# fnordware/j2k

Hardware: AMD Instinct MI355X
Metric: Mpixels/s encode, 8Kx8K 16-bit RGB, 5 DWT levels; DWT HBM GB/s vs roofline (higher is better)
Workload: dtype f32

## Files before the change

### j2k_amd/csrc/encoder.cpp

```cpp
#include <hip/hip_runtime.h>

#include <dlfcn.h>

#include <algorithm>
#include <atomic>
#include <chrono>
#include <condition_variable>
#include <functional>
#include <future>
#include <limits>
#include <cstdio>
#include <cstdlib>
#include <cstring>
#include <memory>
#include <mutex>
#include <thread>
#include <string>
#include <vector>

#include "common.h"
#include "geometry.h"
#include "kernels.h"
#include "tier2.h"
#include "jp2.h"
// ... 625 lines not shown
                hipStream_t side = coder_stream(e, 0);
                HIP_CHECK(hipEventRecord(e->rc_fixed, s));
                HIP_CHECK(hipStreamWaitEvent(side, e->rc_fixed, 0));
                HIP_CHECK(hipMemcpyAsync(e->h_passes.p, ta.pass_nmsedec, tt.h_passes_bytes(), hipMemcpyDeviceToHost, side));
                HIP_CHECK(hipEventRecord(e->rc_tables, side));
                pd.rc_tables_pending = true;
            }
            HIP_CHECK(hipMemcpyAsync(e->h_rc_bounds.p, ra.bounds, 3 * nb * sizeof(double), hipMemcpyDeviceToHost, s));
        }
    } else {
        pd.rc_device = false;
        if (cod.cblk_style && nb) {
            T1Args tf = ta;
            tf.first = 0; tf.nblks = (int)nb;
            launch_t1_rate_fixup(tf, s);
            e->h_passes.ensure(tt.h_rates_bytes());
            HIP_CHECK(hipMemcpyAsync(e->h_passes.p, ta.pass_rate, tt.h_rates_bytes(), hipMemcpyDeviceToHost, s));
        }
    }
    if (overlap_mq) dev.last_dense_done = e->k1_done;
    else HIP_CHECK(hipStreamSynchronize(s));
    dense.unlock();

    pd.active = true;
    pd.F = F; pd.nb1 = nb1; pd.framed = framed; pd.rate_control = rate_control; pd.dwt_bytes = dwt_bytes;
    pd.meta = meta; pd.dblk = dblk; pd.nl = NL;
}

std::vector<EncodeOut> encode_end(j2k_hip_encoder *e)
{
    Pending &pd = e->pend;
    if (!pd.active) throw Error(J2K_HIP_ERR_PARAM, "no encode in progress on this handle");
    if (pd.banded) throw Error(J2K_HIP_ERR_PARAM, "internal: a band-pipelined encode ends in encode_end_banded");
    pd.active = false;
    struct Leave {
        j2k_hip_encoder *e;
        ~Leave() { if (e->counted_inflight) { g_dev[e->device].inflight.fetch_sub(1); e->counted_inflight = false; } }
    } leave{e};
    HIP_CHECK(hipSetDevice(e->device));
    hipStream_t s = e->stream;
    const Geometry &g = e->geo;
    const Coding &cod = g.cod;
    const size_t F = pd.F, nb1 = pd.nb1, nb = nb1 * F;
    const bool framed = pd.framed, rate_control = pd.rate_control;
    const int NL = pd.nl;
    uint32_t *meta = pd.meta;
    const CblkDev *dblk = pd.dblk;
    const std::vector<CblkDev> &hblk = F > 1 ? e->h_blks_seq : e->h_blks;
    {
        Range r("j2k_hip wait t1");
        HIP_CHECK(hipStreamSynchronize(s));
    }
    const double t_t2 = now_ms();
    const T1Tables tt(nb);
    const uint32_t *hm = e->h_meta.as<uint32_t>();
    if (*tt.err(hm) != 0)
        throw Error(J2K_HIP_ERR_OVERFLOW, "Tier-1 kernel reported error " + std::to_string(*tt.err(hm)) +
                                              " (1: too many bit-planes, 2: decision buffer, 3: codeword buffer)");
    uint64_t nsym_total = 0;
    for (size_t i = 0; i < nb; ++i) nsym_total += tt.nsym(hm)[i];
    const size_t lead = main_header(cod).size() + jp2_file_header(cod, 0).size();
    std::vector<Tier2Plan> plans(F);
    std::vector<GatherPlan> lays(F);
    std::vector<size_t> plan_off(F), cs_off(F);
    size_t plan_total = 0, cs_total = 0;
    const size_t nbd = rate_control ? 0 : nb1;
    uint32_t guard = cod.guard;
    {
        Range r("j2k_hip tier2 host");
        for (size_t f = 0; f < F; ++f) {
            std::vector<CblkResult> res(nb1);
            const size_t b0 = f * nb1;
            for (size_t i = 0; i < nb1; ++i) res[i] = CblkResult{tt.numbps(hm)[b0 + i], tt.npasses(hm)[b0 + i], tt.len(hm)[b0 + i]};
            if (cod.cblk_style)
                for (size_t i = 0; i < nb1; ++i) res[i].rates = e->h_passes.as<uint32_t>() + tt.row(b0 + i);
            auto plan_frame = [&](const Geometry &gg) -> Tier2Plan {
                LayerAlloc alloc;
                if (rate_control) {
                    const uint32_t *hp = e->h_passes.as<uint32_t>();
                    const uint32_t *h_rate = tt.h_rate(hp) + tt.row(b0), *h_nmsedec = hp + tt.row(b0);
#ifdef J2K_ALLOC_DUMP
                    if (pd.rc_tables_pending) { HIP_CHECK(hipEventSynchronize(e->rc_tables)); pd.rc_tables_pending = false; }
                    if (const char *path = std::getenv("J2K_ALLOC_DUMP")) {
                        static bool dumped = false;
                        if (!dumped && f == 0) {
                            dumped = true;
                            if (FILE *fp = std::fopen(path, "wb")) {
                                const uint32_t head[10] = {(uint32_t)nb1, (uint32_t)kDevMaxPasses, cod.width, cod.height, cod.ncomp, cod.prec,
                                                           cod.reversible ? 1u : 0u, cod.numres, 1u << cod.cbw, 1u << cod.cbh};
                                std::fwrite(head, 4, 10, fp);
                                for (size_t i = 0; i < nb1; ++i) {
                                    const uint32_t r3[3] = {res[i].numbps, res[i].npasses, res[i].len};
                                    std::fwrite(r3, 4, 3, fp);
                                    std::fwrite(h_rate + tt.row(i), 4, res[i].npasses, fp);
                                    std::fwrite(h_nmsedec + tt.row(i), 4, res[i].npasses, fp);
                                }
                                std::fclose(fp);
                            }
                        }
                    }
#endif
                    std::unique_ptr<HipRateDevice> rdev;
                    if (pd.rc_device) rdev.reset(new HipRateDevice(e, tt));
                    const unsigned at = std::max(1u, std::min((unsigned)std::max(1, tuning().alloc_threads), std::thread::hardware_concurrency()));
                    if (nb1 >= 4096 && !(e->alloc_workers && e->alloc_workers->size() == at)) e->alloc_workers.reset(new Workers(at));
                    alloc = allocate_layers(gg, res, h_rate, reinterpret_cast<const int32_t *>(h_nmsedec), lead, at, rdev.get(), e->alloc_workers.get());
                }
                if (pd.rc_tables_pending) { HIP_CHECK(hipEventSynchronize(e->rc_tables)); pd.rc_tables_pending = false; }
                if (nb1 >= 4096 && !e->t2_workers) e->t2_workers.reset(new Workers(plan_threads()));
                return plan_codestream(gg, res, framed, framed, rate_control ? &alloc : nullptr, e->t2_workers.get());
            };
            guard = cod.guard;
            try { plans[f] = plan_frame(g); }
            catch (const GuardExcess &) {
                if (!cod.guard_auto) throw;
                guard = guard_bits_needed(g, res);
                plans[f] = plan_frame(with_guard_bits(g, guard));
            }
            lays[f] = GatherPlan(plans[f].blob.size(), plans[f].hdr_segs.size(), nbd, plans[f].body_segs.size());
            plan_off[f] = plan_total;
            plan_total += lays[f].total;
            cs_off[f] = cs_total;
            cs_total += round_up(plans[f].total_len + 64, 256);
        }
    }
    const double t_t2_end = now_ms();

    Range r_asm("j2k_hip assemble");
    e->h_plan.ensure(plan_total);
    e->plan.ensure(plan_total);
    e->cs.ensure(cs_total);
    std::vector<GatherArgs> gas(F);
    for (size_t f = 0; f < F; ++f) {
        const Tier2Plan &plan = plans[f];
        const size_t nh = plan.hdr_segs.size(), nseg = plan.body_segs.size();
        uint8_t *hp = e->h_plan.as<uint8_t>() + plan_off[f];
        std::memcpy(hp, plan.blob.data(), plan.blob.size());
        const GatherTables h = lays[f].tables(hp);
        for (size_t i = 0; i < nh; ++i) { h.hdr_dst[i] = plan.hdr_segs[i].dst; h.hdr_src[i] = plan.hdr_segs[i].src; h.hdr_len[i] = plan.hdr_segs[i].len; }
        if (nbd) std::memcpy(h.cblk_dst, plan.cblk_dst.data(), nbd * 8);
        for (size_t i = 0; i < nseg; ++i) {
            const BodySeg &b = plan.body_segs[i];
            h.seg_dst[i] = b.dst; h.seg_src[i] = hblk[f * nb1 + b.cblk].out_off + b.off; h.seg_len[i] = b.len;
        }
        GatherArgs &ga = gas[f];
        lays[f].fill(ga, e->plan.as<uint8_t>() + plan_off[f]);
        ga.dst = e->cs.as<uint8_t>() + cs_off[f];
        ga.out = e->out.as<uint8_t>(); ga.blks = dblk + f * nb1; ga.len = tt.len(meta) + f * nb1; ga.nblks = (int)nbd;
    }
    HIP_CHECK(hipMemcpyAsync(e->plan.p, e->h_plan.p, plan_total, hipMemcpyHostToDevice, s));
    for (size_t f = 0; f < F; ++f) launch_gather(gas[f], s);
    HIP_CHECK(hipEventRecord(e->ev[EV_GATHER], s));
    HIP_CHECK(hipStreamSynchronize(s));

    j2k_hip_stats &st = e->stats;
    st = j2k_hip_stats{};
    float ms = 0;
    HIP_CHECK(hipEventElapsedTime(&ms, e->ev[EV_START], e->ev[EV_UPLOAD])); st.ms_upload = ms;
    HIP_CHECK(hipEventElapsedTime(&ms, e->ev[EV_UPLOAD], e->ev[EV_FRONT])); st.ms_frontend = ms;
    HIP_CHECK(hipEventElapsedTime(&ms, e->ev[EV_FRONT], e->ev[EV_DWT])); st.ms_dwt = ms;
    HIP_CHECK(hipEventElapsedTime(&ms, e->ev[EV_DWT], e->ev[EV_T1])); st.ms_t1 = ms;
    if (tuning().level_events && F == 1) {
        for (int l = 0; l < NL; ++l) { HIP_CHECK(hipEventElapsedTime(&ms, e->lev[l], e->lev[l + 1])); e->level_ms[l] = ms; }
    } else if (NL > 0 && F == 1) {
        HIP_CHECK(hipEventElapsedTime(&ms, e->lev[0], e->lev[1])); e->level_ms[0] = ms;
        if (NL > 1) {
            HIP_CHECK(hipEventElapsedTime(&ms, e->lev[1], e->lev[NL]));
            for (int l = 1; l < NL; ++l) e->level_ms[l] = ms / (NL - 1);
        }
    } else if (NL > 0) {
        HIP_CHECK(hipEventElapsedTime(&ms, e->lev[0], e->lev[NL]));
        for (int l = 0; l < NL; ++l) e->level_ms[l] = ms / NL;
    }
    st.ms_t2_host = t_t2_end - t_t2;
    st.ms_assemble = now_ms() - t_t2_end;
    st.codestream_bytes = 0;
    for (const Tier2Plan &pl : plans) st.codestream_bytes += pl.total_len;
    st.num_codeblocks = nb;
    st.num_symbols = nsym_total;
    st.dwt_bytes = pd.dwt_bytes;
    st.ms_total = now_ms() - pd.t_begin;
    st.ms_after_upload = st.ms_total - st.ms_upload;
    std::vector<EncodeOut> outs(F);
    for (size_t f = 0; f < F; ++f) { outs[f].d_cs = e->cs.as<uint8_t>() + cs_off[f]; outs[f].len = (size_t)plans[f].total_len; }
    if (framed) e->last_guard = guard;
    return outs;
}



void frame_span(const Coding &cod, const j2k_hip_plane *planes, int y0, int y1, const uint8_t *&lo, const uint8_t *&hi)
{
    lo = hi = nullptr;
    for (uint32_t c = 0; c < cod.ncomp; ++c) {
        const j2k_hip_plane &p = planes[c];
        if (!p.base) throw Error(J2K_HIP_ERR_PARAM, "channel buffer is NULL");
        check_plane(cod, p);
        const uint8_t *b = static_cast<const uint8_t *>(p.base);
        const uint8_t *corners[4] = {b + (ptrdiff_t)y0 * p.rowbytes, b + (ptrdiff_t)(y1 - 1) * p.rowbytes,
                                     b + (ptrdiff_t)y0 * p.rowbytes + (ptrdiff_t)(cod.width - 1) * p.colbytes,
                                     b + (ptrdiff_t)(y1 - 1) * p.rowbytes + (ptrdiff_t)(cod.width - 1) * p.colbytes};
        for (const uint8_t *q : corners) {
            if (!lo || q < lo) lo = q;
            if (!hi || q + p.sample_bits / 8 > hi) hi = q + p.sample_bits / 8;
        }
    }
// ... 190 lines not shown
    HIP_CHECK(hipEventRecord(e->ev[EV_T1], s));

    pd.active = true;
    pd.F = 1; pd.nb1 = nb; pd.framed = true; pd.rate_control = false; pd.dwt_bytes = dwt_bytes;
    pd.meta = meta; pd.dblk = ta.blks; pd.nl = NL;
    pd.banded = true; pd.stages = NS; pd.bands = B; pd.ms_upload_host = up_ms;
    return true;
}

struct PieceWriter {
    j2k_hip_write_fn write; void *user; std::vector<uint8_t> &bounce; size_t fill = 0;
    static constexpr size_t kSmall = 256u << 10, kBounce = 4u << 20;
    void out(const uint8_t *p, size_t n) { if (n && write(user, p, n) != n) throw Error(J2K_HIP_ERR_SINK, "Error writing file"); }
    void flush() { if (fill) { out(bounce.data(), fill); fill = 0; } }
    void put(const uint8_t *p, size_t n)
    {
        if (n >= kSmall) { flush(); out(p, n); return; }
        if (bounce.size() < kBounce) bounce.resize(kBounce);
        if (fill + n > kBounce) flush();
        std::memcpy(bounce.data() + fill, p, n);
        fill += n;
    }
};

void encode_end_banded(j2k_hip_encoder *e, j2k_hip_write_fn write, void *user)
{
    Pending &pd = e->pend;
    if (!pd.active || !pd.banded) throw Error(J2K_HIP_ERR_PARAM, "no band-pipelined encode in progress on this handle");
    pd.active = false; pd.banded = false;
    struct Leave {
        j2k_hip_encoder *e;
        ~Leave() { if (e->counted_inflight) { g_dev[e->device].inflight.fetch_sub(1); e->counted_inflight = false; } }
    } leave{e};
    HIP_CHECK(hipSetDevice(e->device));
    const Geometry &g = e->geo;
    const BandSchedule &S = e->band;
    const size_t nb = pd.nb1;
    const int NS = pd.stages, B = pd.bands;
    const T1Tables tt(nb);
    const uint32_t *hm = e->h_meta.as<uint32_t>();
    std::vector<uint64_t> pack_off(nb);
    std::vector<CblkResult> res(nb);
    uint64_t early = 0, nsym_total = 0;
    std::mutex mu;
    std::condition_variable cv;
    uint32_t done_mask = 0;
    bool failed = false;
    const std::function<void(uint32_t)> before_res = [&](uint32_t r) {
        std::unique_lock<std::mutex> lk(mu);
        const uint32_t need = r < S.res_stages.size() ? S.res_stages[r] : 0u;
        cv.wait(lk, [&] { return failed || (done_mask & need) == need; });
        if (failed) throw Error(J2K_HIP_ERR_DEVICE, "the frame's stages did not complete");
    };
    if (nb >= 4096 && !e->t2_workers) e->t2_workers.reset(new Workers(plan_threads()));
    double t_t2 = 0, t_t2_end = 0;
    std::future<Tier2Plan> planner = std::async(std::launch::async, [&] {
        Range r("j2k_hip tier2 host");
        Tier2Plan pl = plan_codestream(g, res, true, true, nullptr, e->t2_workers.get(), &before_res);
        t_t2_end = now_ms();
        return pl;
    });
    auto abandon = [&] {
        { std::lock_guard<std::mutex> lk(mu); failed = true; }
        cv.notify_all();
        try { (void)planner.get(); } catch (...) {}
    };
    try {
        Range r("j2k_hip stages down");
        bool pending[j2k_hip_encoder::kMaxStages] = {};
        int remaining = NS;
        for (int k = 0; k < NS; ++k) pending[k] = true;
        while (remaining) {
            bool progress = false;
            for (int k = 0; k < NS; ++k) {
                if (!pending[k]) continue;
                const hipError_t q = hipEventQuery(e->stage_done[k]);
                if (q == hipErrorNotReady) continue;
                HIP_CHECK(q);
                const BandStage &st = S.stages[(size_t)k];
                uint64_t tot = 0;
                for (size_t n = st.blk_first; n < (size_t)st.blk_first + st.blk_count; ++n) {
                    pack_off[n] = tot; tot += tt.len(hm)[n]; nsym_total += tt.nsym(hm)[n];
                    res[S.perm[n]] = CblkResult{tt.numbps(hm)[n], tt.npasses(hm)[n], tt.len(hm)[n]};
                }
                if (tot) {
                    if (tot > e->out_bytes) throw Error(J2K_HIP_ERR_OVERFLOW, "internal: a stage's codewords exceed the arena");
                    e->h_stage_cs[k].ensure((size_t)tot);
                    HIP_CHECK(hipMemcpyAsync(e->h_stage_cs[k].p, e->cs.as<uint8_t>() + e->h_blks_band[st.blk_first].out_off, (size_t)tot, hipMemcpyDeviceToHost, coder_stream(e, 1)));
                }
                HIP_CHECK(hipEventRecord(e->stage_dl[k], coder_stream(e, 1)));
                if (st.band < B - 1) early += tot;
                { std::lock_guard<std::mutex> lk(mu); done_mask |= 1u << k; }
                cv.notify_all();
                pending[k] = false; --remaining; progress = true;
                if (remaining == 0) t_t2 = now_ms();
            }
            if (!progress) std::this_thread::sleep_for(std::chrono::microseconds(20));
        }
        HIP_CHECK(hipStreamSynchronize(e->stream));
    } catch (...) {
        abandon();
        throw;
    }
    if (*tt.err(hm) != 0) {
        abandon();
        throw Error(J2K_HIP_ERR_OVERFLOW, "Tier-1 kernel reported error " + std::to_string(*tt.err(hm)) +
                                              " (1: too many bit-planes, 2: decision buffer, 3: codeword buffer)");
    }
    Tier2Plan plan;
    uint32_t guard = g.cod.guard;
    try { plan = planner.get(); }
    catch (const GuardExcess &) {
        if (!g.cod.guard_auto) throw;
        Range r("j2k_hip tier2 host, guard bits");
        guard = guard_bits_needed(g, res);
        plan = plan_codestream(with_guard_bits(g, guard), res, true, true, nullptr, e->t2_workers.get());
        t_t2_end = now_ms();
    }
    struct Piece { uint64_t dst; const uint8_t *src; uint64_t len; int stage; };
    std::vector<Piece> hp, bp, all;
    hp.reserve(plan.hdr_segs.size()); bp.reserve(nb);
    for (const HeaderSeg &h : plan.hdr_segs) if (h.len) hp.push_back({h.dst, plan.blob.data() + h.src, h.len, -1});
    for (size_t i = 0; i < nb; ++i) {
        if (!res[i].len) continue;
        const size_t n = S.inv[i];
        const int k = (int)S.stage_of[n];
        const uint8_t *src = e->h_stage_cs[k].as<uint8_t>() + pack_off[n];
        if (!bp.empty() && bp.back().stage == k && bp.back().dst + bp.back().len == plan.cblk_dst[i] && bp.back().src + bp.back().len == src)
            bp.back().len += res[i].len;
        else bp.push_back({plan.cblk_dst[i], src, res[i].len, k});
    }
    auto by_dst = [](const Piece &a, const Piece &b) { return a.dst < b.dst; };
    if (!std::is_sorted(hp.begin(), hp.end(), by_dst)) std::sort(hp.begin(), hp.end(), by_dst);
    if (!std::is_sorted(bp.begin(), bp.end(), by_dst)) std::sort(bp.begin(), bp.end(), by_dst);
    all.resize(hp.size() + bp.size());
    std::merge(hp.begin(), hp.end(), bp.begin(), bp.end(), all.begin(), by_dst);
    {
        Range r("j2k_hip sink");
        PieceWriter w{write, user, e->bounce};
        bool arrived[j2k_hip_encoder::kMaxStages] = {};
        uint64_t pos = 0;
        double waited = 0;
        for (const Piece &pc : all) {
            if (pc.dst != pos) throw Error(J2K_HIP_ERR_PARAM, "internal: the file's pieces do not join up");
            if (pc.stage >= 0 && !arrived[pc.stage]) {
                const double tw = now_ms();
                HIP_CHECK(hipEventSynchronize(e->stage_dl[pc.stage]));
                waited += now_ms() - tw;
                arrived[pc.stage] = true;
            }
            w.put(pc.src, (size_t)pc.len);
            pos += pc.len;
        }
        w.flush();
        if (pos != plan.total_len) throw Error(J2K_HIP_ERR_PARAM, "internal: the file's pieces do not add up to its length");
        e->stats.ms_download = waited;
    }
    HIP_CHECK(hipStreamSynchronize(coder_stream(e, 1)));

    j2k_hip_stats &st = e->stats;
    const double waited = st.ms_download;
    st = j2k_hip_stats{};
    float ms = 0;
    HIP_CHECK(hipEventElapsedTime(&ms, e->ev[EV_START], e->ev[EV_T1]));
    st.ms_t1 = ms;
    st.ms_upload = pd.ms_upload_host;
    st.ms_t2_host = t_t2_end - t_t2;
    st.ms_download = waited;
    st.codestream_bytes = plan.total_len;
// ... 521 lines not shown
```

### j2k_amd/csrc/handle.h

```cpp
#pragma once

#include <hip/hip_runtime.h>

#include <atomic>
#include <chrono>
#include <cstdlib>
#include <future>
#include <memory>
#include <string>
#include <thread>
#include <vector>

#include "bands.h"
#include "common.h"
#include "geometry.h"
#include "kernels.h"
#include "table_layout.h"

namespace j2k_hip {

#define HIP_CHECK(expr)                                                                             \
    do {                                                                                            \
        hipError_t e_ = (expr);                                                                     \
        if (e_ != hipSuccess)                                                                       \
            throw Error(J2K_HIP_ERR_DEVICE, std::string(#expr) + ": " + hipGetErrorString(e_));     \
    } while (0)

struct DevBuf {
    void *p = nullptr;
    size_t cap = 0;
    DevBuf() = default;
    DevBuf(const DevBuf &) = delete;
    DevBuf &operator=(const DevBuf &) = delete;
    ~DevBuf() { release(); }
    void ensure(size_t n)
    {
        if (n <= cap) return;
        if (p) { (void)hipFree(p); p = nullptr; cap = 0; }
        const size_t want = n + n / 8 + 4096;
        if (hipMalloc(&p, want) != hipSuccess) {
            p = nullptr;
            throw Error(J2K_HIP_ERR_MEMORY, "hipMalloc of " + std::to_string(want) + " bytes failed");
        }
        cap = want;
    }
    void release() { if (p) (void)hipFree(p); p = nullptr; cap = 0; }
    template <typename T> T *as() const { return reinterpret_cast<T *>(p); }
};

struct PinnedBuf {
    void *p = nullptr;
    size_t cap = 0;
    PinnedBuf() = default;
    PinnedBuf(const PinnedBuf &) = delete;
    PinnedBuf &operator=(const PinnedBuf &) = delete;
    ~PinnedBuf() { release(); }
    void ensure(size_t n)
    {
        if (n <= cap) return;
        if (p) { (void)hipHostFree(p); p = nullptr; cap = 0; }
        const size_t want = n + n / 8 + 4096;
        if (hipHostMalloc(&p, want, hipHostMallocDefault) != hipSuccess) {
            p = nullptr;
            throw Error(J2K_HIP_ERR_MEMORY, "hipHostMalloc of " + std::to_string(want) + " bytes failed");
        }
        cap = want;
    }
    void release() { if (p) (void)hipHostFree(p); p = nullptr; cap = 0; }
    template <typename T> T *as() const { return reinterpret_cast<T *>(p); }
};

static_assert(kMaxPasses == kDevMaxPasses, "table_layout.h and the Tier-1 kernels agree on the passes per block");

inline unsigned plan_threads() { return std::max(1u, std::min(4u, std::thread::hardware_concurrency())); }

inline int hw_queues()
{
    static const int q = [] {
        const char *v = std::getenv("GPU_MAX_HW_QUEUES");
        const int n = v ? std::atoi(v) : 0;
        return n > 0 ? n : 4;
    }();
    return q;
}

inline double now_ms()
{
    using namespace std::chrono;
    return duration<double, std::milli>(steady_clock::now().time_since_epoch()).count();
}

enum { EV_START, EV_UPLOAD, EV_FRONT, EV_DWT, EV_T1, EV_GATHER, EV_DONE, EV_COUNT };

constexpr int kMaxLevels = 33;


}

struct Pending {
    bool active = false;
    double t_begin = 0;
    size_t F = 1, nb1 = 0;
    bool framed = true, rate_control = false;
    bool rc_device = false;
    bool rc_tables_pending = false;
    double dwt_bytes = 0;
    uint32_t *meta = nullptr;
    const j2k_hip::CblkDev *dblk = nullptr;
    int nl = 0;
    bool banded = false;
    int stages = 0, bands = 0;
    double ms_upload_host = 0, t_uploaded = 0;
};

struct j2k_hip_encoder {
    int device = 0;
    Pending pend;
    std::future<int> begin_job;
    std::atomic<bool> begin_async{false};
    j2k_hip_params begin_params = {};
    j2k_hip_plane begin_planes[4] = {};
    bool last_fused = false;
    j2k_hip::FrontendArgs last_fa = {};
    hipStream_t stream = nullptr;
    hipStream_t mqs[12] = {};
    hipEvent_t gev[12] = {};
    hipEvent_t mq_done[12] = {};
// ... 132 lines not shown
```

### j2k_amd/csrc/kernels.h

```cpp
#pragma once

#include <hip/hip_runtime.h>

#include <cstdint>

#include "rgba_plan.h"

namespace j2k_hip {

struct Tuning {
    int overlap = 1;
    int no_fuse = 0;
    int level_events = 0;
    int level1_dispatch_events = 1;
    int mq_prio = 1;
    int mq_yield = 2;
    int groups = 2;
    int alloc_threads = 8;
    int rate_dev = 0;
    int rate_dev_scan = 0;
    int mq_wait_us = 1500;
    int dwt_pairs = 2;
    int dwt_ppc = 0;
    int dwt_min_waves = 2048;
    int fused_wpb = 0;
    int fused_ppc = 0;
    int fused_generic = 0;
    int dwt_xcd = 1;
    int t1dec_tail = 1;
    int t1dec_lanes = 1;
    int decseq_group = 0;
    int bands = 0;
    int t1_sparse = 0;
};
Tuning &tuning();
int tune(const char *key, int value);
int get_tune(const char *key, int *value);

struct FrontendArgs {
    const uint8_t *src[4];
    long long colbytes[4], rowbytes[4];
    int sample_bytes[4];
    int src_depth[4];
    int ncomp;
    int width;
    int x0;
    int y0, y1;
    int dst_x0, dst_y0;
    int prec;
    int reversible, mct, promote;
    int interleaved;
    const uint8_t *pixel_base;
    int pixel_bytes;
    int chan_off[4];
    void *dst[4];
    long long dst_stride;
    const float *xyz_lin[3];
    const float *xyz_thr;
    float xyz_m[9];
};
void launch_frontend(const FrontendArgs &a, hipStream_t s);
void launch_frontend_sycc(const FrontendArgs &a, int sub_x, int sub_y, hipStream_t s);
void launch_frontend_xyz(const FrontendArgs &a, hipStream_t s);

constexpr int kCompareWords = 8;
constexpr int kCompareSets = 16;
struct CompareArgs {
    FrontendArgs src;
    int wide;
    const int *planes[4]; long long plane_stride; int plane_dc;
    const uint16_t *dec[4]; long long dec_stride[4]; int dec_sx[4], dec_sy[4];
    int ncomp, width, height;
    int slot[4];
    unsigned long long *acc;
};
void launch_compare(const CompareArgs &a, hipStream_t s);

struct DwtJob {
    long long src_off;
    long long ll_off;
    long long z_off;
    int rw, rh;
    int casx, casy;
    int px0, py0;
};
struct DwtLevelArgs {
// ... 202 lines not shown
```

### j2k_amd/csrc/tier2.cpp

```cpp
#include "tier2.h"
#include "cblk_style.h"
#include "jp2.h"

#include <algorithm>
#include <cstring>

namespace j2k_hip {
namespace {

struct ByteVec {
    std::vector<uint8_t> &v;
    void u8(unsigned x) { v.push_back((uint8_t)x); }
    void u16(unsigned x) { u8(x >> 8); u8(x & 0xff); }
    void u32(uint32_t x) { u16(x >> 16); u16(x & 0xffff); }
};

struct BitWriter {
    std::vector<uint8_t> &out;
    uint32_t buf = 0;
    int ct = 8;
    explicit BitWriter(std::vector<uint8_t> &o) : out(o) {}
    void byteout()
    {
        buf = (buf << 8) & 0xffff;
        ct = buf == 0xff00 ? 7 : 8;
        out.push_back((uint8_t)(buf >> 8));
    }
    void bit(unsigned b)
    {
        if (ct == 0) byteout();
        --ct;
        buf |= b << ct;
    }
    void bits(uint32_t v, int n) { for (int i = n - 1; i >= 0; --i) bit((v >> i) & 1); }
    void flush() { byteout(); if (ct == 7) byteout(); }
};

class TagTree {
    struct Node { int parent; int value, low; bool known; };
    std::vector<Node> n_;
  public:
    TagTree(uint32_t w, uint32_t h)
    {
        std::vector<std::pair<uint32_t, uint32_t>> dims;
        uint32_t cw = w, ch = h;
        size_t total = 0;
        while (true) {
            dims.push_back({cw, ch});
            total += (size_t)cw * ch;
            if ((size_t)cw * ch <= 1) break;
            cw = (cw + 1) / 2; ch = (ch + 1) / 2;
        }
        n_.assign(total, Node{-1, 999, 0, false});
        size_t base = 0;
        for (size_t l = 0; l + 1 < dims.size(); ++l) {
            const size_t next = base + (size_t)dims[l].first * dims[l].second;
            for (uint32_t y = 0; y < dims[l].second; ++y)
                for (uint32_t x = 0; x < dims[l].first; ++x)
// ... 707 lines not shown
        }
    };
    if (nt <= 1) packets_of(0); else workers->run(std::min(nt, std::max(1u, npackets)), packets_of);
    uint64_t total = m.committed_bytes;
    if (per_comp) for (uint32_t c = 0; c < m.ncomp; ++c) per_comp[c] = 0;
    for (uint32_t pr = 0; pr < m.pairs.size(); ++pr)
        for (uint32_t pi = m.pairs[pr].packet0; pi < m.pairs[pr].packet0 + m.pairs[pr].npackets; ++pi) {
            total += m.packet_total[pi];
            if (per_comp) per_comp[pr % m.ncomp] += m.packet_total[pi];
        }
    return total;
}

uint64_t TilePricer::committed() const { return p_->committed_bytes; }

uint32_t packet_block_bits(uint32_t np, uint32_t len)
{
    if (!np) return 0;
    BitRecorder r;
    count_numpasses(r, np);
    const int lnp = floorlog2(np);
    const int inc = std::max(0, floorlog2(len) + 1 - (3 + lnp));
    uint32_t bits = (uint32_t)r.n + (uint32_t)inc + 1u;
    return bits + (uint32_t)(3 + inc + lnp);
}

uint64_t TilePricer::tree_bits_bound(uint32_t comp) const
{
    const Impl &m = *p_;
    uint64_t bits = 0;
    for (uint32_t pr = comp; pr < m.pairs.size(); pr += m.ncomp)
        for (uint32_t pi = m.pairs[pr].packet0; pi < m.pairs[pr].packet0 + m.pairs[pr].npackets; ++pi) {
            ++bits;
            for (uint32_t ui = m.packets[pi].unit0; ui < m.packets[pi].unit0 + m.packets[pi].nunits; ++ui) {
            const Impl::Unit &u = m.units[ui];
        for (uint32_t i = u.node0; i < u.node1; ++i) {
            bits += 2;
            const int32_t par = m.parent[i];
            const int v = m.imsb[i].value, pv = par >= 0 ? m.imsb[(size_t)par].value : 0;
            if (v < 999) bits += (uint64_t)(v - pv) + 1u;
        }
            }
        }
    return bits;
}

void TilePricer::commit(const LayerAlloc &alloc, uint32_t layno)
{
    Impl &m = *p_;
    for (const Impl::Pair &pr : m.pairs) m.committed_bytes += m.walk_pair(pr, alloc, layno, m.incl.data(), m.imsb.data(), true);
    m.forget_candidate();
}

Tier2Plan plan_codestream(const Geometry &geo, const std::vector<CblkResult> &res, bool with_main_header,
                          bool with_eoc, const LayerAlloc *alloc, Workers *workers, const std::function<void(uint32_t)> *before_res)
{
    const Coding &cod = geo.cod;
    Tier2Plan plan;
    if (!alloc) plan.cblk_dst.assign(geo.cblks.size(), 0);
    std::vector<uint8_t> &blob = plan.blob;
    blob.reserve(geo.cblks.size() * 4 + 4096);
    uint64_t pos = 0;
    size_t seg_start = 0;
    auto flush_seg = [&]() {
        if (blob.size() > seg_start) {
            plan.hdr_segs.push_back({pos, (uint32_t)seg_start, (uint32_t)(blob.size() - seg_start)});
            pos += blob.size() - seg_start;
            seg_start = blob.size();
        }
    };
    if (blob.capacity() > 0xffffffffull) throw Error(J2K_HIP_ERR_OVERFLOW, "header blob too large");

    if (with_main_header) {
        const std::vector<uint8_t> mh = main_header(cod);
        blob.insert(blob.end(), mh.begin(), mh.end());
    }

    for (const Tile &T : geo.tiles) {
        flush_seg();
        const uint64_t sot_pos = pos;
        const size_t sot_blob = blob.size();
        const uint32_t ntp = cod.dci_tileparts();
        uint64_t tp_sot_pos = sot_pos;
        size_t tp_sot_blob = sot_blob;
        uint32_t cur_tp = 0;
        auto open_tilepart = [&](uint32_t k) {
            flush_seg();
            tp_sot_pos = pos; tp_sot_blob = blob.size(); cur_tp = k;
            ByteVec o{blob};
            o.u16(0xff90); o.u16(10); o.u16(T.index); o.u32(0); o.u8(k); o.u8(ntp);
            o.u16(0xff93);
        };
        auto close_tilepart = [&]() {
            flush_seg();
            const uint64_t psot = pos - tp_sot_pos;
            if (psot > 0xffffffffull) throw Error(J2K_HIP_ERR_OVERFLOW, "tile-part longer than 4 GiB");
            blob[tp_sot_blob + 6] = (uint8_t)(psot >> 24); blob[tp_sot_blob + 7] = (uint8_t)(psot >> 16);
            blob[tp_sot_blob + 8] = (uint8_t)(psot >> 8);  blob[tp_sot_blob + 9] = (uint8_t)psot;
            if (cod.dci && with_main_header) {
                size_t q = 2;
                while (q + 4 <= blob.size() && !(blob[q] == 0xff && blob[q + 1] == 0x55)) q += 2 + (((size_t)blob[q + 2] << 8) | blob[q + 3]);
                const size_t e = q + 6 + 5 * (size_t)cur_tp;
                if (q + 4 > blob.size() || e + 5 > blob.size()) throw Error(J2K_HIP_ERR_OVERFLOW, "TLM segment not found");
                blob[e] = (uint8_t)T.index;
                blob[e + 1] = (uint8_t)(psot >> 24); blob[e + 2] = (uint8_t)(psot >> 16); blob[e + 3] = (uint8_t)(psot >> 8); blob[e + 4] = (uint8_t)psot;
            }
        };
        open_tilepart(0);
        const uint32_t pairs = cod.numres * cod.ncomp;
        const uint32_t nt = workers && T.num_cblks >= 4096 ? std::min<uint32_t>(pairs, workers->size()) : 1u;
        if (nt > 1 || cod.dci) {
            struct Rec { uint32_t hdr_off, hdr_len; uint64_t body_len; uint32_t first, count; };
            struct Piece { uint64_t rel; uint32_t id, off, len; };
            struct PairOut { std::vector<uint8_t> blob; std::vector<Rec> recs; std::vector<Piece> pieces; size_t cursor = 0; };
            std::vector<PairOut> out(pairs);
            auto do_pair = [&](uint32_t p) {
                if (before_res) (*before_res)(p / cod.ncomp);
                PairOut &po = out[p];
                uint64_t body = 0;
                size_t hdr_start = 0;
                uint32_t first = 0;
                bool open = false;
                auto close = [&] { if (open) { po.recs.back().body_len = body; po.recs.back().count = (uint32_t)po.pieces.size() - first; } };
                for_each_packet(cod, T, res, alloc, cod.layers, po.blob,
                                [&] {
                                    close();
                                    po.recs.push_back(Rec{(uint32_t)hdr_start, (uint32_t)(po.blob.size() - hdr_start), 0, (uint32_t)po.pieces.size(), 0});
                                    hdr_start = po.blob.size(); body = 0; first = (uint32_t)po.pieces.size(); open = true;
                                },
                                [&](uint32_t id, uint32_t, uint32_t, uint32_t len, uint32_t off) {
                                    if (!alloc || len) po.pieces.push_back(Piece{body, id, off, len});
                                    body += len;
                                }, p, pairs);
                close();
            };
            if (nt > 1) workers->run(nt, [&](unsigned t) { for (uint32_t k = t; k < pairs; k += nt) do_pair(pairs - 1 - k); });
            else for (uint32_t k = 0; k < pairs; ++k) do_pair(k);
            auto emit = [&](uint32_t r, uint32_t c) {
                PairOut &po = out[(size_t)r * cod.ncomp + c];
                {
                    if (po.cursor >= po.recs.size()) throw Error(J2K_HIP_ERR_OVERFLOW, "packet records out of step");
                    const Rec &rc = po.recs[po.cursor++];
                    blob.insert(blob.end(), po.blob.begin() + rc.hdr_off, po.blob.begin() + rc.hdr_off + rc.hdr_len);
                    flush_seg();
                    for (uint32_t k = rc.first; k < rc.first + rc.count; ++k) {
                        const Piece &pc = po.pieces[k];
                        if (alloc) plan.body_segs.push_back({pos + pc.rel, pc.id, pc.off, pc.len});
                        else plan.cblk_dst[pc.id] = pos + pc.rel;
                    }
                    pos += rc.body_len;
                }
            };
            std::vector<PacketRef> order;
            if (cod.dci == 4)
                order = packet_order_poc(cod, T, cod.layers, {PocEntry{0, 0, 1, cod.numres - 1, cod.ncomp, J2K_HIP_CPRL},
                                                              PocEntry{cod.numres - 1, 0, 1, cod.numres, cod.ncomp, J2K_HIP_CPRL}});
            else order = packet_order(cod, T, cod.layers);
            for (const PacketRef &pr : order) {
                if (cod.dci) {
                    const uint32_t tp = pr.comp + (cod.dci == 4 && pr.res == cod.numres - 1 ? cod.ncomp : 0u);
                    if (tp != cur_tp) { close_tilepart(); open_tilepart(tp); }
                }
                emit(pr.res, pr.comp);
            }
// ... 30 lines not shown
```

### j2k_amd/csrc/tier2.h

```cpp
#pragma once

#include <functional>

#include "geometry.h"

namespace j2k_hip {

struct CblkResult {
    uint32_t numbps;
    uint32_t npasses;
    uint32_t len;
    const uint32_t *rates = nullptr;
};

struct HeaderSeg { uint64_t dst; uint32_t src; uint32_t len; };
struct BodySeg { uint64_t dst; uint32_t cblk; uint32_t off; uint32_t len; };

struct LayerAlloc {
    uint32_t layers = 0;
    std::vector<uint32_t> np, len, off;
};

struct Tier2Plan {
    std::vector<uint8_t> blob;
    std::vector<HeaderSeg> hdr_segs;
    std::vector<uint64_t> cblk_dst;
    std::vector<BodySeg> body_segs;
    uint64_t total_len = 0;
};

uint32_t guard_bits_needed(const Geometry &geo, const std::vector<CblkResult> &res);

std::vector<uint8_t> main_header(const Coding &cod);

Tier2Plan plan_codestream(const Geometry &geo, const std::vector<CblkResult> &res, bool with_main_header,
                          bool with_eoc, const LayerAlloc *alloc = nullptr, Workers *workers = nullptr,
                          const std::function<void(uint32_t)> *before_res = nullptr);

uint64_t tile_packets_size(const Geometry &geo, const Tile &T, const std::vector<CblkResult> &res, const LayerAlloc *alloc,
                           uint32_t maxlayers, Workers *workers = nullptr);
void tile_packets_size_by_comp(const Geometry &geo, const Tile &T, const std::vector<CblkResult> &res, const LayerAlloc *alloc,
                               uint32_t maxlayers, uint64_t *out);

uint32_t packet_block_bits(uint32_t np, uint32_t len);

class TilePricer {
  public:
    TilePricer(const Geometry &geo, const Tile &T, const std::vector<CblkResult> &res);
    ~TilePricer();
    uint64_t price(const LayerAlloc &alloc, uint32_t layno, Workers *workers = nullptr, uint64_t *per_comp = nullptr,
                   const std::vector<uint32_t> *touched = nullptr);
    void commit(const LayerAlloc &alloc, uint32_t layno);
    uint64_t committed() const;
    uint64_t tree_bits_bound(uint32_t comp) const;
  private:
    struct Impl;
    Impl *p_;
};

}
```

### j2k_amd/csrc/tuning.cpp

```cpp
#include <cstdlib>
#include <cstring>
#include <mutex>

#include "kernels.h"

namespace j2k_hip {
namespace {

struct Knob { const char *key; const char *env; int Tuning::*field; };
const Knob kKnobs[] = {
    {"overlap", nullptr, &Tuning::overlap},
    {"no_fuse", "J2K_NO_FUSE", &Tuning::no_fuse},
    {"level_events", "J2K_DWT_LEVEL_EVENTS", &Tuning::level_events},
    {"mq_prio", "J2K_MQ_PRIO", &Tuning::mq_prio},
    {"level1_dispatch_events", "J2K_LEVEL1_DISPATCH_EVENTS", &Tuning::level1_dispatch_events},
    {"groups", "J2K_GROUPS", &Tuning::groups},
    {"mq_wait_us", "J2K_MQ_WAIT_US", &Tuning::mq_wait_us},
    {"dwt_pairs", "J2K_DWT_PAIRS", &Tuning::dwt_pairs},
    {"mq_yield", "J2K_MQ_YIELD", &Tuning::mq_yield},
    {"alloc_threads", "J2K_ALLOC_THREADS", &Tuning::alloc_threads},
    {"rate_dev", "J2K_RATE_DEV", &Tuning::rate_dev},
    {"rate_dev_scan", "J2K_RATE_DEV_SCAN", &Tuning::rate_dev_scan},
    {"dwt_ppc", "J2K_DWT_PPC", &Tuning::dwt_ppc},
    {"dwt_min_waves", "J2K_DWT_MIN_WAVES", &Tuning::dwt_min_waves},
    {"fused_wpb", "J2K_DWT_FUSED_WPB", &Tuning::fused_wpb},
    {"fused_ppc", "J2K_DWT_FUSED_PPC", &Tuning::fused_ppc},
    {"fused_generic", "J2K_DWT_FUSED_GENERIC", &Tuning::fused_generic},
    {"dwt_xcd", "J2K_DWT_XCD", &Tuning::dwt_xcd},
    {"t1dec_lanes", "J2K_T1DEC_LANES", &Tuning::t1dec_lanes},
    {"t1dec_tail", "J2K_T1DEC_TAIL", &Tuning::t1dec_tail},
    {"decseq_group", "J2K_DECSEQ_GROUP", &Tuning::decseq_group},
    {"bands", "J2K_BANDS", &Tuning::bands},
    {"t1_sparse", "J2K_T1_SPARSE", &Tuning::t1_sparse},
};

Tuning g_tuning;
std::once_flag g_once;

void from_env()
{
    for (const Knob &k : kKnobs) {
        if (!k.env) continue;
        const char *v = std::getenv(k.env);
        if (v && *v) g_tuning.*(k.field) = std::atoi(v);
        else if (v && (k.field == &Tuning::no_fuse || k.field == &Tuning::level_events))
            g_tuning.*(k.field) = 1;
    }
    if (std::getenv("J2K_NO_OVERLAP")) g_tuning.overlap = 0;
}

}

Tuning &tuning()
{
    std::call_once(g_once, from_env);
    return g_tuning;
}

int tune(const char *key, int value)
{
    if (!key) return 1;
    Tuning &t = tuning();
    for (const Knob &k : kKnobs)
        if (std::strcmp(k.key, key) == 0) { t.*(k.field) = value; return 0; }
    return 1;
}

int get_tune(const char *key, int *value)
{
    if (!key || !value) return 1;
    Tuning &t = tuning();
    for (const Knob &k : kKnobs)
        if (std::strcmp(k.key, key) == 0) { *value = t.*(k.field); return 0; }
    return 1;
}

}
```

Before: 10760.

## Add parallel plain Tier-2 packet header writer with word-level bit packing

```diff
diff --git a/j2k_amd/csrc/encoder.cpp b/j2k_amd/csrc/encoder.cpp
--- a/j2k_amd/csrc/encoder.cpp
+++ b/j2k_amd/csrc/encoder.cpp
@@ -701,6 +701,8 @@
         HIP_CHECK(hipStreamSynchronize(s));
     }
     const double t_t2 = now_ms();
+    static const bool tail_trace = std::getenv("J2K_TAIL_TRACE") != nullptr;
+    double ms_res = 0, ms_plan = 0;
     const T1Tables tt(nb);
     const uint32_t *hm = e->h_meta.as<uint32_t>();
     if (*tt.err(hm) != 0)
@@ -718,9 +720,11 @@
     {
         Range r("j2k_hip tier2 host");
         for (size_t f = 0; f < F; ++f) {
+            const double t_res = now_ms();
             std::vector<CblkResult> res(nb1);
             const size_t b0 = f * nb1;
             for (size_t i = 0; i < nb1; ++i) res[i] = CblkResult{tt.numbps(hm)[b0 + i], tt.npasses(hm)[b0 + i], tt.len(hm)[b0 + i]};
+            ms_res += now_ms() - t_res;
             if (cod.cblk_style)
                 for (size_t i = 0; i < nb1; ++i) res[i].rates = e->h_passes.as<uint32_t>() + tt.row(b0 + i);
             auto plan_frame = [&](const Geometry &gg) -> Tier2Plan {
@@ -756,16 +760,18 @@
                     alloc = allocate_layers(gg, res, h_rate, reinterpret_cast<const int32_t *>(h_nmsedec), lead, at, rdev.get(), e->alloc_workers.get());
                 }
                 if (pd.rc_tables_pending) { HIP_CHECK(hipEventSynchronize(e->rc_tables)); pd.rc_tables_pending = false; }
-                if (nb1 >= 4096 && !e->t2_workers) e->t2_workers.reset(new Workers(plan_threads()));
-                return plan_codestream(gg, res, framed, framed, rate_control ? &alloc : nullptr, e->t2_workers.get());
+                if (nb1 >= 4096 && !e->t2_workers) e->t2_workers.reset(new Workers(t2_threads()));
+                return plan_codestream(gg, res, framed, framed, rate_control ? &alloc : nullptr, e->t2_workers.get(), nullptr, tuning().t2_writer);
             };
             guard = cod.guard;
+            const double t_plan = now_ms();
             try { plans[f] = plan_frame(g); }
             catch (const GuardExcess &) {
                 if (!cod.guard_auto) throw;
                 guard = guard_bits_needed(g, res);
                 plans[f] = plan_frame(with_guard_bits(g, guard));
             }
+            ms_plan += now_ms() - t_plan;
             lays[f] = GatherPlan(plans[f].blob.size(), plans[f].hdr_segs.size(), nbd, plans[f].body_segs.size());
             plan_off[f] = plan_total;
             plan_total += lays[f].total;
@@ -797,10 +803,15 @@
         ga.dst = e->cs.as<uint8_t>() + cs_off[f];
         ga.out = e->out.as<uint8_t>(); ga.blks = dblk + f * nb1; ga.len = tt.len(meta) + f * nb1; ga.nblks = (int)nbd;
     }
+    const double t_copied = now_ms();
     HIP_CHECK(hipMemcpyAsync(e->plan.p, e->h_plan.p, plan_total, hipMemcpyHostToDevice, s));
     for (size_t f = 0; f < F; ++f) launch_gather(gas[f], s);
     HIP_CHECK(hipEventRecord(e->ev[EV_GATHER], s));
+    const double t_launched = now_ms();
     HIP_CHECK(hipStreamSynchronize(s));
+    if (tail_trace)
+        std::fprintf(stderr, "j2k_hip tail: results %.3f ms, plan %.3f, rest of tier-2 %.3f | plan copy %.3f, upload + gather launches %.3f, wait %.3f\n",
+                     ms_res, ms_plan, t_t2_end - t_t2 - ms_res - ms_plan, t_copied - t_t2_end, t_launched - t_copied, now_ms() - t_launched);
 
     j2k_hip_stats &st = e->stats;
     st = j2k_hip_stats{};
@@ -1097,11 +1108,12 @@
         cv.wait(lk, [&] { return failed || (done_mask & need) == need; });
         if (failed) throw Error(J2K_HIP_ERR_DEVICE, "the frame's stages did not complete");
     };
-    if (nb >= 4096 && !e->t2_workers) e->t2_workers.reset(new Workers(plan_threads()));
+    if (nb >= 4096 && !e->t2_workers) e->t2_workers.reset(new Workers(t2_threads()));
     double t_t2 = 0, t_t2_end = 0;
+    const int t2_writer = tuning().t2_writer;
     std::future<Tier2Plan> planner = std::async(std::launch::async, [&] {
         Range r("j2k_hip tier2 host");
-        Tier2Plan pl = plan_codestream(g, res, true, true, nullptr, e->t2_workers.get(), &before_res);
+        Tier2Plan pl = plan_codestream(g, res, true, true, nullptr, e->t2_workers.get(), &before_res, t2_writer);
         t_t2_end = now_ms();
         return pl;
     });
@@ -1159,7 +1171,7 @@
         if (!g.cod.guard_auto) throw;
         Range r("j2k_hip tier2 host, guard bits");
         guard = guard_bits_needed(g, res);
-        plan = plan_codestream(with_guard_bits(g, guard), res, true, true, nullptr, e->t2_workers.get());
+        plan = plan_codestream(with_guard_bits(g, guard), res, true, true, nullptr, e->t2_workers.get(), nullptr, t2_writer);
         t_t2_end = now_ms();
     }
     struct Piece { uint64_t dst; const uint8_t *src; uint64_t len; int stage; };
diff --git a/j2k_amd/csrc/handle.h b/j2k_amd/csrc/handle.h
--- a/j2k_amd/csrc/handle.h
+++ b/j2k_amd/csrc/handle.h
@@ -73,6 +73,11 @@
 static_assert(kMaxPasses == kDevMaxPasses, "table_layout.h and the Tier-1 kernels agree on the passes per block");
 
 inline unsigned plan_threads() { return std::max(1u, std::min(4u, std::thread::hardware_concurrency())); }
+inline unsigned t2_threads()
+{
+    const int n = tuning().t2_threads;
+    return n > 0 ? std::max(1u, std::min({(unsigned)n, 16u, std::thread::hardware_concurrency()})) : plan_threads();
+}
 
 inline int hw_queues()
 {
diff --git a/j2k_amd/csrc/kernels.h b/j2k_amd/csrc/kernels.h
--- a/j2k_amd/csrc/kernels.h
+++ b/j2k_amd/csrc/kernels.h
@@ -32,6 +32,8 @@
     int decseq_group = 0;
     int bands = 0;
     int t1_sparse = 0;
+    int t2_writer = 0;
+    int t2_threads = 0;
 };
 Tuning &tuning();
 int tune(const char *key, int value);
diff --git a/j2k_amd/csrc/tier2.cpp b/j2k_amd/csrc/tier2.cpp
--- a/j2k_amd/csrc/tier2.cpp
+++ b/j2k_amd/csrc/tier2.cpp
@@ -3,7 +3,10 @@
 #include "jp2.h"
 
 #include <algorithm>
+#include <atomic>
 #include <cstring>
+#include <memory>
+#include <thread>
 
 namespace j2k_hip {
 namespace {
@@ -817,10 +820,331 @@
     m.forget_candidate();
 }
 
+namespace {
+
+constexpr uint32_t kPlainPiece = 1024;
+
+struct PlainUnit {
+    uint32_t first_cblk, cw, ch, res, node0, nlev;
+    int Mb;
+};
+struct PlainPiece { uint32_t unit, k0, k1, packet; std::vector<uint64_t> words; uint64_t nbits = 0, body = 0; };
+struct PlainPacket { uint32_t piece0 = 0, npieces = 0; std::unique_ptr<uint8_t[]> hdr; size_t hdr_len = 0; uint64_t body = 0; };
+
+struct BitAcc {
+    uint64_t *at;
+    uint64_t acc = 0;
+    int room = 64;
+    void put(uint64_t x, int len)
+    {
+        if (len <= room) { room -= len; acc |= x << room; return; }
+        const int over = len - room;
+        *at++ = acc | (x >> over);
+        room = 64 - over;
+        acc = x << room;
+    }
+};
+
+inline int ilog2(uint32_t a) { return a > 1 ? 31 - __builtin_clz(a) : 0; }
+
+size_t stuff_stream(const uint64_t *w, uint64_t nbits, uint8_t *out, std::vector<uint64_t> *ff)
+{
+    uint8_t *o = out;
+    uint64_t pos = 0;
+    bool after_ff = false;
+    auto peek = [&](uint64_t p) {
+        const size_t i = (size_t)(p >> 6);
+        const int s = (int)(p & 63);
+        return s ? (w[i] << s) | (w[i + 1] >> (64 - s)) : w[i];
+    };
+    for (;;) {
+        const uint64_t left = nbits - pos;
+        if (after_ff) {
+            if (left < 7) break;
+            *o++ = (uint8_t)(peek(pos) >> 57);
+            pos += 7; after_ff = false;
+            continue;
+        }
+        if (left >= 64) {
+            const uint64_t x = peek(pos), v = ~x;
+            const uint64_t nz = (((v & 0x7f7f7f7f7f7f7f7full) + 0x7f7f7f7f7f7f7f7full) | v) & 0x8080808080808080ull;
+            const uint64_t be = __builtin_bswap64(x);
+            std::memcpy(o, &be, 8);
+            if (nz == 0x8080808080808080ull) { pos += 64; o += 8; continue; }
+            const int idx = __builtin_clzll(~nz & 0x8080808080808080ull) >> 3;
+            if (ff) ff->push_back(pos + 8ull * (unsigned)idx);
+            pos += 8ull * (unsigned)(idx + 1); o += idx + 1; after_ff = true;
+            continue;
+        }
+        if (left < 8) break;
+        const uint8_t byte = (uint8_t)(peek(pos) >> 56);
+        *o++ = byte;
+        after_ff = byte == 0xffu;
+        if (after_ff && ff) ff->push_back(pos);
+        pos += 8;
+    }
+    if (nbits - pos > 0 || after_ff) *o++ = (uint8_t)(peek(pos) >> (after_ff ? 57 : 56));
+    return (size_t)(o - out);
+}
+
+struct PlainTile {
+    const Coding &cod;
+    const Tile &T;
+    const std::vector<CblkResult> &res;
+    const std::function<void(uint32_t)> *before_res;
+    Tier2Probe *probe;
+    uint64_t *cblk_dst;
+    std::vector<PlainUnit> units;
+    std::vector<PlainPiece> pieces;
+    std::vector<PlainPacket> packets;
+    std::vector<uint32_t> pair_packet0;
+    std::unique_ptr<uint8_t[]> zb, inc;
+    std::unique_ptr<uint32_t[]> first;
+    std::unique_ptr<std::atomic<uint32_t>[]> filled, left;
+    struct Task { uint32_t fill, idx; };
+    std::vector<Task> tasks;
+    std::atomic<uint32_t> next{0};
+    std::atomic<bool> failed{false};
+
+    PlainTile(const Coding &c, const Tile &t, const std::vector<CblkResult> &r, const std::function<void(uint32_t)> *br, Tier2Probe *pb,
+              uint64_t *dst, uint32_t piece)
+        : cod(c), T(t), res(r), before_res(br), probe(pb), cblk_dst(dst)
+    {
+        size_t nodes = 0;
+        std::vector<uint32_t> res_unit0(cod.numres + 1, 0), res_piece0(cod.numres + 1, 0);
+        pair_packet0.resize((size_t)cod.numres * cod.ncomp);
+        for (uint32_t r = 0; r < cod.numres; ++r) {
+            for (uint32_t c = 0; c < cod.ncomp; ++c) {
+                const Resolution &R = T.comps[c].res[r];
+                pair_packet0[(size_t)r * cod.ncomp + c] = (uint32_t)packets.size();
+                for (uint32_t pn = 0; pn < R.pw * R.ph; ++pn) {
+                    PlainPacket pk;
+                    pk.piece0 = (uint32_t)pieces.size();
+                    for (uint32_t b = 0; b < R.nbands; ++b) {
+                        const Band &B = R.bands[b];
+                        if (B.empty()) continue;
+                        const Precinct &P = B.precs[pn];
+                        const uint32_t n = P.cw * P.ch;
+                        if (!n) continue;
+                        PlainUnit u{P.first_cblk, P.cw, P.ch, r, (uint32_t)nodes, 0, B.q.numbps};
+                        for (uint32_t w = P.cw, h = P.ch;; w = (w + 1) / 2, h = (h + 1) / 2) {
+                            nodes += (size_t)w * h; ++u.nlev;
+                            if ((size_t)w * h <= 1) break;
+                        }
+                        const uint32_t np = (n + piece - 1) / piece, each = (n + np - 1) / np;
+                        for (uint32_t k0 = 0; k0 < n; k0 += each) {
+                            PlainPiece pc;
+                            pc.unit = (uint32_t)units.size(); pc.k0 = k0; pc.k1 = std::min(n, k0 + each); pc.packet = (uint32_t)packets.size();
+                            pieces.push_back(std::move(pc));
+                        }
+                        units.push_back(u);
+                    }
+                    pk.npieces = (uint32_t)pieces.size() - pk.piece0;
+                    packets.push_back(std::move(pk));
+                }
+            }
+            res_unit0[r + 1] = (uint32_t)units.size(); res_piece0[r + 1] = (uint32_t)pieces.size();
+        }
+        if (nodes > 0xffffffffull) throw Error(J2K_HIP_ERR_OVERFLOW, "tag trees too large");
+        zb.reset(new uint8_t[nodes]); inc.reset(new uint8_t[nodes]); first.reset(new uint32_t[nodes]);
+        filled.reset(new std::atomic<uint32_t>[units.size() + 1]);
+        left.reset(new std::atomic<uint32_t>[packets.size() + 1]);
+        for (size_t i = 0; i < units.size(); ++i) filled[i].store(0, std::memory_order_relaxed);
+        for (size_t i = 0; i < packets.size(); ++i) left[i].store(packets[i].npieces, std::memory_order_relaxed);
+        tasks.reserve(units.size() + pieces.size());
+        for (uint32_t r = cod.numres; r-- > 0;) {
+            for (uint32_t i = res_unit0[r]; i < res_unit0[r + 1]; ++i) tasks.push_back(Task{1, i});
+            for (uint32_t i = res_piece0[r]; i < res_piece0[r + 1]; ++i) tasks.push_back(Task{0, i});
+        }
+    }
+
+    void fill(const PlainUnit &u)
+    {
+        if (before_res) (*before_res)(u.res);
+        uint8_t *z = zb.get() + u.node0, *in = inc.get() + u.node0;
+        uint32_t *f = first.get() + u.node0;
+        const uint32_t n = u.cw * u.ch;
+        for (uint32_t k = 0; k < n; ++k) {
+            const CblkResult &r = res[u.first_cblk + k];
+            const int zbp = u.Mb - (int)r.numbps;
+            if (zbp < 0) throw GuardExcess();
+            z[k] = (uint8_t)std::min(zbp, 255);
+            in[k] = r.npasses != 0;
+            f[k] = r.npasses ? k : ~0u;
+        }
+        uint32_t w = u.cw, h = u.ch;
+        size_t lo = 0;
+        for (uint32_t l = 1; l < u.nlev; ++l) {
+            const uint32_t pw = (w + 1) / 2, ph = (h + 1) / 2;
+            const size_t up = lo + (size_t)w * h;
+            for (uint32_t y = 0; y < ph; ++y)
+                for (uint32_t x = 0; x < pw; ++x) {
+                    const size_t a = lo + (size_t)(2 * y) * w + 2 * x;
+                    uint8_t zv = z[a], iv = in[a];
+                    uint32_t fv = f[a];
+                    auto child = [&](size_t c) { zv = std::min(zv, z[c]); iv |= in[c]; fv = std::min(fv, f[c]); };
+                    if (2 * x + 1 < w) child(a + 1);
+                    if (2 * y + 1 < h) { child(a + w); if (2 * x + 1 < w) child(a + w + 1); }
+                    const size_t d = up + (size_t)y * pw + x;
+                    z[d] = zv; in[d] = iv; f[d] = fv;
+                }
+            lo = up; w = pw; h = ph;
+        }
+    }
+
+    void write(PlainPiece &pc)
+    {
+        const PlainUnit &u = units[pc.unit];
+        const uint8_t *z = zb.get() + u.node0, *in = inc.get() + u.node0;
+        const uint32_t *f = first.get() + u.node0;
+        uint32_t W[34];
+        size_t O[34];
+        {
+            uint32_t w = u.cw, h = u.ch;
+            size_t o = 0;
+            for (uint32_t l = 0; l < u.nlev; ++l) { W[l] = w; O[l] = o; o += (size_t)w * h; w = (w + 1) / 2; h = (h + 1) / 2; }
+        }
+        const int top = (int)u.nlev - 1;
+        auto node = [&](int l, uint32_t x, uint32_t y) { return O[l] + (size_t)(y >> l) * W[l] + (x >> l); };
+        const size_t ahead = ((size_t)u.nlev * 40 + 87) / 64 + 2;
+        pc.words.resize((size_t)(pc.k1 - pc.k0) + ahead);
+        BitAcc a{pc.words.data()};
+        uint64_t run = 0;
+        uint32_t x = pc.k0 % u.cw, y = pc.k0 / u.cw;
+        for (uint32_t k = pc.k0; k < pc.k1; ++k) {
+            const CblkResult &r = res[u.first_cblk + k];
+            const uint32_t np = r.npasses;
+            if ((size_t)(a.at - pc.words.data()) + ahead > pc.words.size()) {
+                const size_t done = (size_t)(a.at - pc.words.data());
+                pc.words.resize(pc.words.size() * 2);
+                a.at = pc.words.data() + done;
+            }
+            const int m = (x | y) ? std::min(__builtin_ctz(x | y), top) : top;
+            if (np) a.put((2ull << m) - 1ull, m + 1);
+            else if (m == top || in[node(m + 1, x, y)])
+                for (int l = m; l >= 0; --l) {
+                    const unsigned b = in[node(l, x, y)];
+                    a.put(b, 1);
+                    if (!b) break;
+                }
+            if (np) {
+                int m2 = 0;
+                while (m2 < top && f[node(m2 + 1, x, y)] == k) ++m2;
+                for (int l = m2; l >= 0; --l) {
+                    const int v = z[node(l, x, y)], pv = l < top ? z[node(l + 1, x, y)] : 0;
+                    a.put(1, v - pv + 1);
+                }
+                const uint32_t len = r.len;
+                const int lnp = ilog2(np), up = std::max(0, ilog2(len) + 1 - (3 + lnp));
+                uint64_t code;
+                int cn;
+                if (np == 1) { code = 0; cn = 1; }
+                else if (np == 2) { code = 2; cn = 2; }
+                else if (np <= 5) { code = 0xc | (np - 3); cn = 4; }
+                else if (np <= 36) { code = 0x1e0 | (np - 6); cn = 9; }
+                else { code = 0xff80 | (np - 37); cn = 16; }
+                a.put((code << (up + 1)) | ((1ull << (up + 1)) - 2ull), cn + up + 1);
+                a.put(len, 3 + up + lnp);
+                cblk_dst[u.first_cblk + k] = run;
+                run += len;
+            } else cblk_dst[u.first_cblk + k] = ~0ull;
+            if (++x == u.cw) { x = 0; ++y; }
+        }
+        pc.nbits = (uint64_t)(a.at - pc.words.data()) * 64u + (uint64_t)(64 - a.room);
+        if (a.room < 64) *a.at++ = a.acc;
+        pc.body = run;
+    }
+
+    void finish(uint32_t p)
+    {
+        PlainPacket &pk = packets[p];
+        uint64_t nbits = 1;
+        for (uint32_t i = pk.piece0; i < pk.piece0 + pk.npieces; ++i) nbits += pieces[i].nbits;
+        const size_t nw = (size_t)((nbits + 63) >> 6);
+        const std::unique_ptr<uint64_t[]> all(new uint64_t[nw + 3]);
+        uint64_t *w = all.get();
+        w[0] = 1ull << 63;
+        uint64_t at = 1;
+        std::vector<uint64_t> splices;
+        for (uint32_t i = pk.piece0; i < pk.piece0 + pk.npieces; ++i) {
+            PlainPiece &pc = pieces[i];
+            if (probe && i > pk.piece0) splices.push_back(at);
+            const size_t n = (size_t)((pc.nbits + 63) >> 6), d = (size_t)(at >> 6);
+            const int s = (int)(at & 63);
+            if (!s) { std::memcpy(w + d, pc.words.data(), n * 8); if (n) w[d + n] = 0; }
+            else for (size_t j = 0; j < n; ++j) { w[d + j] |= pc.words[j] >> s; w[d + j + 1] = pc.words[j] << (64 - s); }
+            at += pc.nbits;
+            pk.body += pc.body;
+            std::vector<uint64_t>().swap(pc.words);
+        }
+        w[nw] = w[nw + 1] = w[nw + 2] = 0;
+        std::vector<uint64_t> ff;
+        pk.hdr.reset(new uint8_t[(size_t)(nbits / 7) + 16]);
+        pk.hdr_len = stuff_stream(w, nbits, pk.hdr.get(), probe ? &ff : nullptr);
+        if (probe)
+            for (const uint64_t at : ff) {
+                const auto s = std::upper_bound(splices.begin(), splices.end(), at);
+                if (s != splices.end() && *s < at + 8) probe->ff_splice[*s & 63].fetch_add(1);
+                else probe->ff_inside.fetch_add(1);
+                if (at + 8 >= nbits) probe->ff_last.fetch_add(1);
+            }
+    }
+
+    void run_task(const Task &t)
+    {
+        if (t.fill) {
+            fill(units[t.idx]);
+            filled[t.idx].store(1, std::memory_order_release);
+            return;
+        }
+        PlainPiece &pc = pieces[t.idx];
+        if (before_res) (*before_res)(units[pc.unit].res);
+        while (!filled[pc.unit].load(std::memory_order_acquire)) {
+            if (failed.load(std::memory_order_relaxed)) return;
+            std::this_thread::yield();
+        }
+        write(pc);
+        if (left[pc.packet].fetch_sub(1, std::memory_order_acq_rel) == 1) finish(pc.packet);
+    }
+
+    void run(Workers *workers, uint32_t nt)
+    {
+        for (uint32_t p = 0; p < packets.size(); ++p) if (!packets[p].npieces) finish(p);
+        auto work = [&](unsigned) {
+            try {
+                for (;;) {
+                    const uint32_t i = next.fetch_add(1, std::memory_order_relaxed);
+                    if (i >= tasks.size() || failed.load(std::memory_order_relaxed)) break;
+                    run_task(tasks[i]);
+                }
+            } catch (...) {
+                failed.store(true, std::memory_order_relaxed);
+                throw;
+            }
+        };
+        if (nt > 1) workers->run(nt, work); else work(0);
+    }
+
+    void place(uint32_t p, uint64_t base)
+    {
+        const PlainPacket &pk = packets[p];
+        for (uint32_t i = pk.piece0; i < pk.piece0 + pk.npieces; ++i) {
+            const PlainPiece &pc = pieces[i];
+            uint64_t *d = cblk_dst + units[pc.unit].first_cblk;
+            for (uint32_t k = pc.k0; k < pc.k1; ++k) d[k] = d[k] == ~0ull ? 0 : d[k] + base;
+            base += pc.body;
+        }
+    }
+};
+
+}
+
 Tier2Plan plan_codestream(const Geometry &geo, const std::vector<CblkResult> &res, bool with_main_header,
-                          bool with_eoc, const LayerAlloc *alloc, Workers *workers, const std::function<void(uint32_t)> *before_res)
+                          bool with_eoc, const LayerAlloc *alloc, Workers *workers, const std::function<void(uint32_t)> *before_res,
+                          int writer, Tier2Probe *probe)
 {
     const Coding &cod = geo.cod;
+    const bool plain = writer >= 0 && !alloc && cod.layers == 1 && !cod.cblk_style && !cod.dci;
     Tier2Plan plan;
     if (!alloc) plan.cblk_dst.assign(geo.cblks.size(), 0);
     std::vector<uint8_t> &blob = plan.blob;
@@ -874,7 +1198,21 @@
         open_tilepart(0);
         const uint32_t pairs = cod.numres * cod.ncomp;
         const uint32_t nt = workers && T.num_cblks >= 4096 ? std::min<uint32_t>(pairs, workers->size()) : 1u;
-        if (nt > 1 || cod.dci) {
+        if (plain) {
+            PlainTile pt(cod, T, res, before_res, probe, plan.cblk_dst.data(), writer > 0 ? (uint32_t)writer : kPlainPiece);
+            pt.run(workers, workers && T.num_cblks >= 4096 ? workers->size() : 1u);
+            size_t hdr_bytes = 0;
+            for (const PlainPacket &pk : pt.packets) hdr_bytes += pk.hdr_len;
+            blob.reserve(blob.size() + hdr_bytes + 16);
+            for (const PacketRef &pr : packet_order(cod, T, cod.layers)) {
+                const uint32_t p = pt.pair_packet0[(size_t)pr.res * cod.ncomp + pr.comp] + pr.prec;
+                const PlainPacket &pk = pt.packets[p];
+                blob.insert(blob.end(), pk.hdr.get(), pk.hdr.get() + pk.hdr_len);
+                flush_seg();
+                pt.place(p, pos);
+                pos += pk.body;
+            }
+        } else if (nt > 1 || cod.dci) {
             struct Rec { uint32_t hdr_off, hdr_len; uint64_t body_len; uint32_t first, count; };
             struct Piece { uint64_t rel; uint32_t id, off, len; };
             struct PairOut { std::vector<uint8_t> blob; std::vector<Rec> recs; std::vector<Piece> pieces; size_t cursor = 0; };
diff --git a/j2k_amd/csrc/tier2.h b/j2k_amd/csrc/tier2.h
--- a/j2k_amd/csrc/tier2.h
+++ b/j2k_amd/csrc/tier2.h
@@ -1,5 +1,6 @@
 #pragma once
 
+#include <atomic>
 #include <functional>
 
 #include "geometry.h"
@@ -33,9 +34,15 @@
 
 std::vector<uint8_t> main_header(const Coding &cod);
 
+struct Tier2Probe {
+    std::atomic<uint64_t> ff_inside{0};
+    std::atomic<uint64_t> ff_last{0};
+    std::atomic<uint64_t> ff_splice[64];
+    Tier2Probe() { for (auto &c : ff_splice) c.store(0); }
+};
 Tier2Plan plan_codestream(const Geometry &geo, const std::vector<CblkResult> &res, bool with_main_header,
                           bool with_eoc, const LayerAlloc *alloc = nullptr, Workers *workers = nullptr,
-                          const std::function<void(uint32_t)> *before_res = nullptr);
+                          const std::function<void(uint32_t)> *before_res = nullptr, int writer = 0, Tier2Probe *probe = nullptr);
 
 uint64_t tile_packets_size(const Geometry &geo, const Tile &T, const std::vector<CblkResult> &res, const LayerAlloc *alloc,
                            uint32_t maxlayers, Workers *workers = nullptr);
diff --git a/j2k_amd/csrc/tuning.cpp b/j2k_amd/csrc/tuning.cpp
--- a/j2k_amd/csrc/tuning.cpp
+++ b/j2k_amd/csrc/tuning.cpp
@@ -32,6 +32,8 @@
     {"decseq_group", "J2K_DECSEQ_GROUP", &Tuning::decseq_group},
     {"bands", "J2K_BANDS", &Tuning::bands},
     {"t1_sparse", "J2K_T1_SPARSE", &Tuning::t1_sparse},
+    {"t2_writer", "J2K_T2_WRITER", &Tuning::t2_writer},
+    {"t2_threads", "J2K_T2_THREADS", &Tuning::t2_threads},
 };
 
 Tuning g_tuning;
```

Result: no change. 10740 (-0.1%).
